# fabriziosestito/policy-server

Measured on AMD Instinct MI355X. Metric: admission requests evaluated/sec (node) at 64 policies; HBM GB/s vs peak, higher is better.
Workload: dtype u8; 1 GPU; C4: 1000000 synthetic Pod AdmissionReviews per GPU x 64 compiled policies (c4_64.yml: 22 psp-capabilities, 21 psp-apparmor, 21 safe-labels); config=c4_64, total_requests=1000000, policies=64, parallelism=dp1 (request shards)

## Files before the change

include/kwgpu.h:

```cpp
#ifndef KWGPU_H
#define KWGPU_H

#include <stddef.h>
#include <stdint.h>

#ifdef __cplusplus
extern "C" {
#endif

enum {
  KW_OK = 0,
  KW_E_INVALID_ID = 1,
  KW_E_INIT = 2,
  KW_E_NOT_FOUND = 3,
  KW_E_BOOTSTRAP = 4,
  KW_E_ENGINE = 5,
  KW_E_GROUP_REHYDRATE = 6,
  KW_E_ARG = 16,
  KW_E_PAYLOAD = 17,
  KW_E_DEVICE = 18,
  KW_E_NOSPACE = 19
};

enum { KW_MODE_PROTECT = 0, KW_MODE_MONITOR = 1 };
// ... 106 lines not shown
int kw_env_pattern_count(const kw_env *env, int col);
int kw_env_pattern(const kw_env *env, int col, int idx, int *kind, char *buf, size_t cap);
int kw_env_classify(const kw_env *env, int col, const char *key, size_t klen, const char *s, size_t len,
                    uint32_t *pats, int cap);

typedef struct kw_batch kw_batch;

int kw_batch_from_json(const char *const *docs, const size_t *lens, size_t n, int doc_kind,
                       kw_batch **out, int64_t *bad_row, char *err, size_t errlen);
int kw_batch_from_soa(const kw_soa *soa, kw_batch **out);
int kw_batch_view(const kw_batch *b, kw_soa *view);
int kw_batch_to_device(kw_batch *b, int device);
int kw_batch_to_device_async(kw_batch *b, int device, void *stream);
int kw_stream_create(int device, void **stream);
void kw_stream_destroy(void *stream);
void kw_batch_destroy(kw_batch *b);

int kw_debug_host_walk(const kw_env *env, const kw_batch *b, const int32_t *policies, uint32_t npol,
                       int origin, uint32_t *out);

int kw_debug_plan(const kw_env *env, kw_batch *b, const int32_t *policies, uint32_t npol, int origin, uint32_t *out,
                  int cap);

int kw_debug_reorder(const kw_batch *b, uint64_t *perm, size_t cap, uint64_t *split, kw_batch **out);

int kw_validate_batch(const kw_env *env, kw_batch *b, const int32_t *policies, uint32_t npol,
                      int origin, void *stream);
int kw_validate_rows(const kw_env *env, kw_batch *b, const int32_t *row_policy, int origin,
                     void *stream);
int kw_batch_verdicts(kw_batch *b, uint32_t *host_out, size_t count);
int kw_validate_host(const kw_env *env, kw_batch *b, const int32_t *policies, uint32_t npol, int origin,
                     int device, uint32_t *out, size_t count, uint32_t chunk_rows);
int kw_batch_pin_host(kw_batch *b, int device);
int kw_host_alloc(int device, size_t bytes, void **out);
void kw_host_free(void *p);
int kw_batch_wide_arg(const kw_batch *b, uint64_t row, int32_t policy, uint64_t *value);
int kw_batch_group_causes(const kw_batch *b, uint64_t row, int32_t policy, uint32_t verdict, uint64_t *words,
                          size_t nwords, size_t *needed);

typedef struct kw_timing {
  double classify_ms;
  double evaluate_ms;
  double total_ms;
  double classify_bytes;
  double evaluate_bytes;
} kw_timing;
// ... 33 lines not shown
```

policy-server_amd/csrc/capi.cpp:

```cpp
#include <hip/hip_runtime.h>

#include <algorithm>
#include <cstdio>
#include <cstdlib>
#include <cstring>
#include <memory>
#include <string>
#include <thread>
#include <vector>

#include "../../include/kwgpu.h"
#include "automaton.hpp"
#include "batch.hpp"
#include "devbatch.hpp"
#include "env.hpp"
#include "kernels.hpp"
#include "knobs.hpp"
#include "metrics.hpp"
#include "pass.hpp"
#include "plan.hpp"
#include "service.hpp"
#include "slotplan.hpp"
#include "upload.hpp"
#include "yaml.hpp"
// ... 512 lines not shown
  std::unique_ptr<DeviceBatch> saved = std::move(kb->dev);
  kb->dev = host_view(kb);
  PassPlan plan;
  int rc = plan_pass(env, kb, policies, npol, nullptr, origin, Knobs::on<KW_BULK_DEBUG>(), &plan);
  const TileArgs& T = plan.geom;
  const uint32_t vals[8] = {T.lds_bytes, (uint32_t)plan.launches.size(), (uint32_t)plan.chunks.size(), T.lds_tables,
                            T.rows, T.cmax, T.kmax, T.lmax};
  for (int i = 0; i < 8; ++i) out[i] = rc == KW_OK ? vals[i] : 0u;
  if (cap >= 16) {
    const bool two = rc == KW_OK && plan.regions.size() == 2;
    const TileArgs* H = two ? &plan.regions[1].geom : nullptr;
    uint32_t more[8] = {rc == KW_OK ? (uint32_t)plan.regions.size() : 0u, (uint32_t)kb->dev->split,
                              rc == KW_OK ? plan.regions[0].grid : 0u, H ? H->lds_bytes : 0u, H ? H->rows : 0u,
                              H ? H->cmax : 0u, two ? plan.regions[1].grid : 0u, 0u};
    if (rc == KW_OK)
      for (size_t k = 0; k < plan.regions.size() && k < 32; ++k) more[7] |= (plan.regions[k].geom.feat & kFeatRng) ? 1u << k : 0u;
    for (int i = 0; i < 8; ++i) out[8 + i] = more[i];
  }
  kb->dev->verdicts = nullptr;
  kb->dev = std::move(saved);
  return rc;
}

int kw_debug_reorder(const kw_batch* kb, uint64_t* perm, size_t cap, uint64_t* split, kw_batch** out) {
  if (!kb || !split || !out || (!perm && kb->b.n) || cap < kb->b.n) return KW_E_ARG;
  std::vector<uint64_t> p;
  *split = split_rows(kb->b, &p);
  if (!*split) {
    p.resize(kb->b.n);
    for (uint64_t r = 0; r < kb->b.n; ++r) p[r] = r;
  }
  auto nb = std::make_unique<kw_batch>();
  RowOrder o;
  permute_batch(kb->b, p, &nb->b, true, &o);
  std::copy(p.begin(), p.end(), perm);
  *out = nb.release();
  return KW_OK;
}

int kw_batch_group_causes(const kw_batch* b, uint64_t row, int32_t policy, uint32_t verdict, uint64_t* words,
                          size_t nwords, size_t* needed) {
  if (!b || (!words && nwords)) return KW_E_ARG;
  if (KW_REASON(verdict) != KW_R_GROUP) return KW_E_ARG;
  const WideData& W = b->b.wide;
  uint32_t bw = 0;
  const uint64_t* big = W.lookup_big(row, policy, &bw);
// ... 128 lines not shown
```

policy-server_amd/csrc/kernels.hip:

```cpp
#include <hip/hip_runtime.h>

#include <algorithm>
#include <array>
#include <cstddef>
#include <mutex>

#include "../../include/kwgpu.h"
#include "imgscan.hpp"
#include "kernels.hpp"


namespace kw {

typedef uint32_t u32x4 __attribute__((ext_vector_type(4)));

__device__ inline uint32_t lit_word(const uint32_t* base, uint32_t i, uint32_t sh, uint32_t len) {
  const uint32_t w = align_bytes(base[i + 1], base[i], sh);
  const uint32_t rem = len - 4u * i;
  return rem >= 4u ? w : (w & ((1u << (8u * rem)) - 1u));
}

template <bool BATCH, int N = 8>
__device__ inline uint32_t lit_lookup(const uint8_t* rec, const uint8_t* bytes, uint32_t b, uint32_t e) {
  const DevLit* L = (const DevLit*)rec;
// ... 337 lines not shown
  x |= (first + 8u <= i) ? y : 0ull;
  y = dpp64<0x142, 0xa>(x);
  x |= (first + r + 1u <= i) ? y : 0ull;
  y = dpp64<0x143, 0xc>(x);
  x |= (lane >= 32u && first + lane - 31u <= i) ? y : 0ull;
  y = dpp64<0x138, 0xf>(x);
  return (first + 1u <= i) ? y : 0ull;
}

template <class T>
__device__ inline const __attribute__((address_space(1))) T* gp(const T* p) {
  return (const __attribute__((address_space(1))) T*)p;
}

__device__ inline uint32_t rup64(uint32_t n) { return (n + 63u) & ~63u; }

__device__ inline uint32_t str_g0(int m, uint32_t r0, uint32_t cb, uint32_t kab, uint32_t kdb, uint32_t lb) {
  return m == S_NS ? r0 : m == S_CAPADD ? kab : m == S_CAPDROP ? kdb : (m == S_LK || m == S_LV) ? lb : cb;
}
__device__ inline uint32_t str_n(int m, uint32_t nr, uint32_t nc, uint32_t nka, uint32_t nkd, uint32_t nl) {
  return m == S_NS ? nr : m == S_CAPADD ? nka : m == S_CAPDROP ? nkd : (m == S_LK || m == S_LV) ? nl : nc;
}

__device__ inline void glds_dwords(const uint32_t* src, uint32_t* dst, uint32_t n, uint32_t tid) {
  const uint32_t lane = tid & 63u;
  for (uint32_t i = tid; i < n; i += kSlotThreads)
    __builtin_amdgcn_global_load_lds((const __attribute__((address_space(1))) void*)(src + i),
                                     (__attribute__((address_space(3))) void*)(dst + (i - lane)), 4, 0, 0);
}
__device__ inline void glds_x4(const u32x4* src, u32x4* dst, uint32_t n, uint32_t tid) {
  const uint32_t lane = tid & 63u;
  for (uint32_t i = tid; i < n; i += kSlotThreads)
    __builtin_amdgcn_global_load_lds((const __attribute__((address_space(1))) void*)(src + i),
                                     (__attribute__((address_space(3))) void*)(dst + (i - lane)), 16, 0, 0);
}
__device__ inline void wglds_dwords(const uint32_t* src, uint32_t* dst, uint32_t n, uint32_t lane) {
  for (uint32_t i = lane; i < n; i += 64u)
    __builtin_amdgcn_global_load_lds((const __attribute__((address_space(1))) void*)(src + i),
                                     (__attribute__((address_space(3))) void*)(dst + (i - lane)), 4, 0, 0);
}
__device__ inline void wglds_x4(const u32x4* src, u32x4* dst, uint32_t n, uint32_t lane) {
  for (uint32_t i = lane; i < n; i += 64u)
    __builtin_amdgcn_global_load_lds((const __attribute__((address_space(1))) void*)(src + i),
                                     (__attribute__((address_space(3))) void*)(dst + (i - lane)), 16, 0, 0);
}

__device__ inline void lds_barrier() { asm volatile("s_waitcnt lgkmcnt(0)\n\ts_barrier" ::: "memory"); }

__device__ inline void prefetch_l2(const void* src, uint32_t bytes, uint8_t* scratch, uint32_t tid) {
  const uint8_t* p = (const uint8_t*)src;
  if ((tid & 63u) >= kPfLanes) return;
  const uint32_t q = (tid >> 6) * kPfLanes + (tid & (kPfLanes - 1u));
// ... 108 lines not shown
  uint32_t* l_cadd = (uint32_t*)region(t.o_cadd);
  uint32_t* l_cdrop = (uint32_t*)region(t.o_cdrop);
  uint16_t* c_ns = (uint16_t*)region(t.o_ns);
  uint16_t* c_aa = (uint16_t*)region(t.o_aa);
  uint16_t* c_img = (uint16_t*)region(t.o_img);
  uint16_t* c_add = (uint16_t*)region(t.o_capadd);
  uint16_t* c_drop = (uint16_t*)region(t.o_capdrop);
  uint16_t* c_lk = (uint16_t*)region(t.o_lk);
  uint16_t* c_lv = (uint16_t*)region(t.o_lv);
  uint64_t* l_rej = (uint64_t*)region(t.o_rej);
  uint64_t* l_mut = (uint64_t*)region(t.o_mut);
  uint8_t* l_byp = region(t.o_byp);
  uint32_t* l_sa = (uint32_t*)region(t.o_sa);
  uint64_t* l_vadd = (uint64_t*)region(t.o_vadd);
  uint64_t* l_vl = (uint64_t*)region(t.o_vl);
  uint64_t* l_vc = (uint64_t*)region(t.o_vc);
  uint64_t* l_vtr = (uint64_t*)region(t.o_vtr);
  uint32_t* l_vw = (uint32_t*)region(t.o_vw);
  uint8_t* own_c = region(t.o_own_c);
  uint8_t* own_l = region(t.o_own_l);
  const ImgLayout il = t.il;
  const uint32_t nim = il.n(), nlv = t.nlv;
  const uint32_t need = t.need;

  if (!desc_early) {
    if (tile < t_hi) fetch_desc(tile, 0);
    __syncthreads();
  }
  mark(4);
  for (uint32_t it = 0; tile < t_hi; ++it) {
    const uint64_t p0_t0 = timing ? clock64() : 0;
    const uint32_t cur = it & 1u;
    uint32_t nxt2 = 0;
    if (dyn && tid == 0) nxt2 = atomicAdd(cnt, 1u);
    if (next < t_hi) fetch_desc(next, cur ^ 1u);
    const TileDesc& d = l_desc[cur];
#define KW_DF(x) sfield(x)
    if (!KW_DF(d.fits)) {
      if (dyn && tid == 0) l_nx[cur] = nxt2;
      __syncthreads();
      tile = next;
      next = dyn ? dbase + l_nx[cur] : next + wpx;
      continue;
    }
    const uint64_t r0 = ((uint64_t)KW_DF(d.r0hi) << 32) | KW_DF(d.r0lo);
    const uint32_t nr = KW_DF(d.nr);
    const uint32_t cb = KW_DF(d.cb), ce = KW_DF(d.ce), lb = KW_DF(d.lb), le = KW_DF(d.le);
    const uint32_t kab = KW_DF(d.kab), kae = KW_DF(d.kae), kdb = KW_DF(d.kdb), kde = KW_DF(d.kde);
    const uint32_t nc = ce - cb, nl = le - lb;
    uint64_t p0_t1 = 0, p0_t2 = 0;
    if (timing) {
      p0_t1 = clock64();
      sg_add(SG_P0_TOP, p0_t1 - p0_t0);
    }

    constexpr bool p0_spread = (LBL || CTR);
    if constexpr (p0_spread) {
      auto job = [&](uint32_t j) { return wave == (j & 3u); };
      if (job(0)) wglds_dwords((const uint32_t*)(a.req_flags + r0), (uint32_t*)l_rf, (nr + 3u) >> 2, lane);
      if (job(1)) wglds_dwords(a.ctr_off + r0, l_coff, nr + 1, lane);
      if (job(2)) wglds_dwords(a.lbl_off + r0, l_loff, nr + 1, lane);
      if (job(3)) wglds_dwords((const uint32_t*)a.ctr_flags + (cb >> 2), (uint32_t*)l_cflags, ((ce + 3u) >> 2) - (cb >> 2), lane);
      if (job(4)) wglds_dwords(a.capadd_off + cb, l_cadd, nc + 1, lane);
      if (job(5)) wglds_dwords(a.capdrop_off + cb, l_cdrop, nc + 1, lane);
      if (timing) {
        p0_t2 = clock64();
        sg_add(SG_P0_REQ, p0_t2 - p0_t1);
      }
#pragma unroll
      for (int m = 0; m < (int)NSTR; ++m) {
        const uint32_t jo = 6u + 2u * (uint32_t)m, jb = jo + 1u;
        if (!(job(jo) || job(jb)) || !t.o_sb[m]) continue;
        if (job(jo)) {
          const uint32_t g0 = str_g0(m, (uint32_t)r0, cb, kab, kdb, lb);
          const uint32_t n = str_n(m, nr, nc, kae - kab, kde - kdb, nl);
          wglds_dwords(t.s_off[m] + g0, (uint32_t*)(lds + t.o_so[m]), n + 1, lane);
        } else {
          wglds_x4((const u32x4*)(t.s_bytes[m] + KW_DF(d.sa[m])), (u32x4*)(lds + t.o_sb[m]), KW_DF(d.nv[m]), lane);
        }
      }
    } else {
      glds_dwords((const uint32_t*)(a.req_flags + r0), (uint32_t*)l_rf, (nr + 3u) >> 2, tid);
      glds_dwords(a.ctr_off + r0, l_coff, nr + 1, tid);
      glds_dwords(a.lbl_off + r0, l_loff, nr + 1, tid);
      glds_dwords((const uint32_t*)a.ctr_flags + (cb >> 2), (uint32_t*)l_cflags, ((ce + 3u) >> 2) - (cb >> 2), tid);
      glds_dwords(a.capadd_off + cb, l_cadd, nc + 1, tid);
      glds_dwords(a.capdrop_off + cb, l_cdrop, nc + 1, tid);
      if (timing) {
        p0_t2 = clock64();
        sg_add(SG_P0_REQ, p0_t2 - p0_t1);
      }
#pragma unroll
      for (int m = 0; m < (int)NSTR; ++m) {
        if (!t.o_sb[m]) continue;
        const uint32_t g0 = str_g0(m, (uint32_t)r0, cb, kab, kdb, lb);
        const uint32_t n = str_n(m, nr, nc, kae - kab, kde - kdb, nl);
        glds_dwords(t.s_off[m] + g0, (uint32_t*)(lds + t.o_so[m]), n + 1, tid);
        glds_x4((const u32x4*)(t.s_bytes[m] + KW_DF(d.sa[m])), (u32x4*)(lds + t.o_sb[m]), KW_DF(d.nv[m]), tid);
      }
    }
    if (timing) sg_add(SG_P0_STR, clock64() - p0_t2);
    for (uint32_t i = tid; i < nr; i += kSlotThreads) l_rej[i] = l_mut[i] = 0;
    if (DYNB && tid == 0) l_nx[2] = l_nx[3] = 0;
    if (tid < NSTR) l_sa[tid] = d.sa[tid];
#undef KW_DF
    const uint64_t p0_end = timing ? clock64() : 0;
    __syncthreads();
    if (timing) sg_add(SG_P0_WAIT, clock64() - p0_end);
    mark(0);
    if (timing && tid == 0) ++ph[5];
    if (dyn && tid == 0) l_nx[cur] = nxt2;
    auto prefetch_next = [&]() {
      if (KW_PREFETCH && LDST && IMG && t.prefetch && next < t_hi) {
        const TileDesc& dn = l_desc[cur ^ 1u];
        if (sfield(dn.fits)) {
          const uint64_t q0 = ((uint64_t)sfield(dn.r0hi) << 32) | sfield(dn.r0lo);
          const uint32_t qn = sfield(dn.nr), qcb = sfield(dn.cb), qc = sfield(dn.ce) - qcb;
          const uint32_t qlb = sfield(dn.lb), qkab = sfield(dn.kab), qkdb = sfield(dn.kdb);
          uint8_t* scratch = lds + t.o_pf;
          prefetch_l2(a.req_flags + q0, qn, scratch, tid);
          prefetch_l2(a.ctr_off + q0, (qn + 1) * 4u, scratch, tid);
          prefetch_l2(a.lbl_off + q0, (qn + 1) * 4u, scratch, tid);
          prefetch_l2(a.ctr_flags + qcb, qc, scratch, tid);
          prefetch_l2(a.capadd_off + qcb, (qc + 1) * 4u, scratch, tid);
// ... 962 lines not shown
```

policy-server_amd/csrc/kernels.hpp:

```cpp
#pragma once
#include <hip/hip_runtime.h>

#include <cstdint>

#include "kwdev.hpp"
#include "slots.hpp"

namespace kw {

enum Str : uint32_t { S_NS = 0, S_IMG, S_AA, S_CAPADD, S_CAPDROP, S_LK, S_LV, NSTR };

struct WideRec {
  uint32_t row_lo, row_hi, policy, value;
};

struct EvalArgs {
  const uint8_t* blob;
  uint64_t nrows;
  uint64_t ndesc;
  uint32_t npol;
  int32_t origin;
  const uint8_t* req_flags;
  const uint32_t* ctr_off;
  const uint32_t* lbl_off;
// ... 30 lines not shown
constexpr uint32_t lds_workgroups_per_cu(uint32_t bytes) {
  const uint32_t g = (bytes + kLdsGranule - 1) / kLdsGranule;
  return g ? kLdsGranules / g : kLdsGranules;
}
constexpr uint32_t kFeatImg = 1, kFeatLbl = 2, kFeatCtr = 4, kFeatGrp = 8, kFeatAll = 15;
constexpr uint32_t kFeatNfa = 16;
constexpr uint32_t kFeatRng = 32;
#ifndef KW_PREFETCH
#define KW_PREFETCH 1
#endif
#ifndef KW_PF_LANES
#define KW_PF_LANES 64
#endif
constexpr uint32_t kPfLanes = KW_PF_LANES;
constexpr uint32_t kMaxChunks = 8;

struct ChunkArgs {
  const uint8_t* rec;
  uint32_t o_lds;
  uint32_t col0, ncols, vec4;
  uint64_t init;
};

struct TileArgs {
  uint32_t rows;
  uint32_t cmax, kmax, lmax;
  uint32_t o_rf, o_coff, o_loff, o_cflags, o_cadd, o_cdrop;
  uint32_t o_ns, o_aa, o_img, o_capadd, o_capdrop, o_lk, o_lv;
  ImgLayout il;
  uint32_t nlv;
  uint32_t need;
  uint32_t o_vadd, o_vl, o_vc, o_vtr;
  uint32_t o_own_c, o_own_l;
  uint32_t o_rej, o_mut, o_byp;
  uint32_t o_nx;
  uint32_t o_desc;
  uint32_t o_pf;
  uint32_t prefetch;
  uint32_t feat;
  uint32_t ctr_ranges;
  uint32_t o_sa;
  uint32_t o_vw, vw_stride;
  uint32_t o_so[NSTR], o_sb[NSTR], sb_cap[NSTR];
  const uint32_t* s_off[NSTR];
  const uint8_t* s_bytes[NSTR];
  uint32_t lds_tables;
  uint32_t lit_lds[NCOL], dfa_lds[NCOL], kv_lds;
  uint32_t lit_blob[NCOL], dfa_blob[NCOL], kv_blob, nlk;
  uint32_t nstage;
  uint32_t stage_blob[NCOL + kMaxChunks], stage_lds[NCOL + kMaxChunks], stage_bytes[NCOL + kMaxChunks];
  uint32_t bypass_cls, docker_io_cls, latest_cls;
  uint32_t nchunk;
  ChunkArgs chunk[kMaxChunks];
  uint32_t rows_mode;
  uint32_t debug;
  uint32_t lds_bytes;
};

struct alignas(16) TileDesc {
  uint32_t cb, ce, lb, le, kab, kae, kdb, kde;
  uint32_t sa[NSTR];
  uint32_t pad0;
  uint32_t nv[NSTR];
  uint32_t fits;
  uint32_t r0lo, r0hi, nr;
  uint32_t pad[4];
};
static_assert(sizeof(TileDesc) == 128, "TileDesc layout");

hipError_t launch_evaluate_tiles(const EvalArgs& a, const TileArgs& t, const TileArgs* d_t, const TileDesc* d_desc,
                                 uint32_t grid, hipStream_t s);
struct WideGroupArgs {
  uint32_t prog_off, prog_len;
  uint32_t col;
  uint32_t nmem, midx_off;
  uint32_t okw, rejb;
  uint32_t cause_off, cause_words;
  uint32_t errw;
  uint32_t kind;
  uint32_t mutw;
};

constexpr uint32_t kSplitMember = 0x80000000u;

template <class Part>
KW_HD inline uint32_t combine_parts(const WideGroupArgs& g, const uint32_t* part_off, Part part) {
  bool mutated = false;
  for (uint32_t s = 0; s < g.nmem; ++s) {
    const uint32_t x = part(s);
    if (!(x & KW_V_ALLOWED)) {
      uint32_t reason = KW_REASON(x), arg = KW_ARG(x);
// ... 55 lines not shown
```

policy-server_amd/csrc/pass.cpp:

```cpp
#include "pass.hpp"

#include <atomic>
#include <chrono>
#include <cstdio>
#include <cstring>
#include <memory>

#include "knobs.hpp"
#include "plan.hpp"

namespace kw {

int upload_env(kw_env* env, int device) {
  if (device < 0) return KW_OK;
  HIPCHK(hipSetDevice(device));
  HIPCHK(hipMalloc(&env->e.d_blob, env->e.blob.size()));
  HIPCHK(hipMemcpy(env->e.d_blob, env->e.blob.data(), env->e.blob.size(), hipMemcpyHostToDevice));
  env->e.device = device;
  return KW_OK;
}

int build_descs(const Batch& B, const TileArgs& T, uint64_t lo, uint64_t hi, uint64_t t0, uint64_t t1, uint64_t range,
                std::vector<TileDesc>* desc, std::vector<uint32_t>* ovf) {
  auto make = [&](uint64_t r0, uint64_t r1, TileDesc* dp) {
// ... 246 lines not shown
  D.last_nwide = plan.nwide;
  D.last_wide_policy = plan.wide_policy;
  D.last_rows_mode = plan.rows_mode;
  D.last_row_words = plan.args.npol;
  D.last_wide_cap = A.wide_cap;
  *out_args = A;
  return KW_OK;
}

static void print_phase_report(size_t launch, uint32_t grid, const std::vector<uint64_t>& ph) {
  double sum[kPhaseWords] = {0};
  for (uint32_t g = 0; g < grid; ++g)
    for (uint32_t k = 0; k < kPhaseWords; ++k) sum[k] += (double)ph[(size_t)g * kPhaseWords + k];
  const double tiles = std::max(1.0, sum[5]);
  fprintf(stderr,
          "[kw phase] launch %zu grid %u tiles %.0f: cycles/tile P0 %.0f P1 %.0f D %.0f P2 %.0f P3+next %.0f "
          "(sum %.0f); per workgroup: %.0f cycles, %.2f tiles, table staging %.0f\n",
          launch, grid, tiles, sum[0] / tiles, sum[1] / tiles, sum[2] / tiles, sum[3] / tiles, sum[4] / tiles,
          (sum[0] + sum[1] + sum[2] + sum[3] + sum[4]) / tiles, sum[6] / grid, tiles / grid, sum[7] / grid);
  const double wt = tiles * (double)(kSlotThreads / 64u);
  const double* g = sum + 8;
  fprintf(stderr,
          "[kw seg] per wave-tile: P0 wait %.0f | P1 busy %.0f wait %.0f (label %.0f capstr %.0f ctr %.0f image %.0f req %.0f) "
          "| P2 busy %.0f wait %.0f (ctr %.0f label %.0f req %.0f) | P3 busy %.0f wait %.0f | P0 issue: top %.0f "
          "request arrays %.0f strings %.0f\n",
          g[SG_P0_WAIT] / wt, g[SG_P1_BUSY] / wt, g[SG_P1_WAIT] / wt, g[SG_P1_LABEL] / wt, g[SG_P1_CAPSTR] / wt,
          g[SG_P1_CTR] / wt, g[SG_P1_IMAGE] / wt, g[SG_P1_REQ] / wt, g[SG_P2_BUSY] / wt, g[SG_P2_WAIT] / wt,
          g[SG_P2_CTR] / wt, g[SG_P2_LABEL] / wt, g[SG_P2_REQ] / wt, g[SG_P3_BUSY] / wt, g[SG_P3_WAIT] / wt,
          g[SG_P0_TOP] / wt, g[SG_P0_REQ] / wt, g[SG_P0_STR] / wt);
  const uint32_t nx = std::min(8u, grid);
  uint32_t late = 0;
  double spread = 0;
  for (uint32_t x = 0; x < nx; ++x) {
    std::vector<uint64_t> st;
    for (uint32_t q = x; q < grid; q += nx) st.push_back(ph[(size_t)q * kPhaseWords + 8 + SG_START]);
    std::sort(st.begin(), st.end());
    for (uint64_t v : st) late += v > st[0] + 2000;
    spread = std::max(spread, (double)(st.back() - st[0]) / 100.0);
  }
  fprintf(stderr, "[kw start] launch %zu: %u of %u workgroups started > 20 us after their XCD's first (widest spread %.1f us)\n",
          launch, late, grid, spread);
}

static int run_pass(kw_batch* kb, PassPlan& plan, bool timed, hipStream_t s) {
  DeviceBatch& D = *kb->dev;
  EvalArgs A;
  if (int rc = prepare_pass(kb, plan, s, &A)) return rc;
  const bool phases = (plan.geom.debug & 512u) != 0;
// ... 272 lines not shown
```

policy-server_amd/csrc/plan.cpp:

```cpp
#define KW_PLANNING_TU
#include "plan.hpp"

#include <algorithm>
#include <chrono>
#include <cstdio>
#include <cstring>
#include <map>

#include "knobs.hpp"
#include "slots.hpp"

namespace kw {

bool sched_dynamic(uint64_t ntiles, uint32_t grid, bool lds_tables) {
  const char* e = PlanKnobs::str<KW_SCHED>();
  if (!strcmp(e, "static")) return false;
  if (!strcmp(e, "dynamic")) return true;
  return ntiles > (lds_tables ? 16ull : 4ull) * std::max<uint32_t>(grid, 1);
}

namespace {

uint32_t heavy_rows() { return (uint32_t)PlanKnobs::num<KW_HEAVY_ROWS>(); }

// ... 543 lines not shown
      T.stage_blob[T.nstage] = stages[k].blob;
      T.stage_lds[T.nstage] = lds_at[k];
      T.stage_bytes[T.nstage] = (stages[k].bytes + 15u) & ~15u;
      ++T.nstage;
    }
  for (int c = 0; c < (int)NCOL; ++c) {
    if (P.lit_of[c]) {
      T.lit_blob[c] = stages[P.lit_of[c] - 1].blob;
      T.lit_lds[c] = lds_at[P.lit_of[c] - 1];
    }
    if (P.dfa_of[c]) {
      T.dfa_blob[c] = stages[P.dfa_of[c] - 1].blob;
      T.dfa_lds[c] = lds_at[P.dfa_of[c] - 1];
    }
  }
  if (P.kv_stage) {
    T.kv_blob = stages[P.kv_stage - 1].blob;
    T.kv_lds = ldst ? lds_at[P.kv_stage - 1] : 0u;
  } else if (need & (1u << S_LV)) {
    T.kv_blob = H->kv_off;
    T.kv_lds = 0;
  }
  T.debug = debug;
}

void dump_plan(const TileArgs& T, const PassNeeds& N, const TablePlan& P, size_t nchunks, size_t nlaunches) {
  fprintf(stderr, "[kw tile] lds_tables=%u rows=%u cmax=%u kmax=%u lmax=%u lds=%u area=%u (classifiers %u) chunks=%zu launches=%zu nim=%u nlv=%u\n",
          T.lds_tables, T.rows, T.cmax, T.kmax, T.lmax, T.lds_bytes, P.area, P.table_bytes, nchunks, nlaunches, N.il.n(), N.nlv);
  for (size_t k = 0; k < P.stages.size(); ++k) fprintf(stderr, "[kw tile]   classifier stage %zu: %u bytes\n", k, P.stages[k].bytes);
  uint32_t so = 0, sb = 0;
  for (int m = 0; m < (int)NSTR; ++m)
    if (T.o_sb[m]) so += T.o_sb[m] - T.o_so[m], sb += T.sb_cap[m] + 48;
  fprintf(stderr,
          "[kw tile]   layout: headers %u | classes ns %u aa %u img %u caps %u lk %u lv %u | sets vadd %u vl %u vc %u vtr %u | "
          "owners %u | rej/mut/byp %u | union at %u: string offsets %u + bytes %u, violation words %u | total %u\n",
          T.o_ns - T.o_rf, T.o_aa - T.o_ns, T.o_img - T.o_aa, T.o_capadd - T.o_img, T.o_lk - T.o_capadd, T.o_lv - T.o_lk,
          T.o_vadd - T.o_lv, T.o_vl - T.o_vadd, T.o_vc - T.o_vl, T.o_vtr - T.o_vc, T.o_own_c - T.o_vtr, T.o_rej - T.o_own_c,
          T.o_sa - T.o_rej, T.o_vw, so, sb, T.rows * T.vw_stride * 4, T.lds_bytes);
}

void plan_launch_args(const TablePlan& P, uint32_t npol, PassPlan* plan) {
  plan->slot_blob.clear();
  plan->slot_at.clear();
  for (const SlotChunk& c : plan->chunks) {
    plan->slot_at.push_back((uint32_t)plan->slot_blob.size());
    plan->slot_blob.insert(plan->slot_blob.end(), c.rec.begin(), c.rec.end());
// ... 32 lines not shown
  A.lbl_off = D.lbl_off;
  A.ctr_flags = D.ctr_flags;
  A.capadd_off = D.capadd_off;
  A.capdrop_off = D.capdrop_off;
  A.out = D.verdicts;
  A.nwide = plan->nwide;
  plan->wide_cap_per_row = plan->rows_mode ? 1u : npol;
  if (!A.req_flags || !A.ctr_off || !A.lbl_off || !A.ctr_flags || !A.capadd_off || !A.capdrop_off || !A.out) return KW_E_ARG;
  for (int m = 0; m < (int)NSTR; ++m)
    if ((N.need & (1u << m)) && (!plan->geom.s_off[m] || !plan->geom.s_bytes[m])) return KW_E_ARG;

  const double n = (double)B.n;
  double eb = n * (1 + 4 + 4) + 4.0 * n * (double)A.npol;
  if (N.any_ctr) eb += (double)B.containers() * 1.0;
  if (N.any_caps) eb += (double)B.containers() * 8.0;
  for (int m = 0; m < (int)NSTR; ++m)
    if (N.need & (1u << m)) eb += (double)D.str[m].nbytes + 4.0 * (double)D.str[m].n;
  plan->evaluate_bytes = eb;
  return KW_OK;
}

}

int plan_pass(const kw_env* env, kw_batch* kb, const int32_t* pols, uint32_t npol, const int32_t* row_policy,
              int origin, bool timing, PassPlan* plan) {
  const Env& E = env->e;
  DeviceBatch& D = *kb->dev;
  const Batch& B = dev_rows(kb);
  const DevHeader* H = (const DevHeader*)E.blob.data();
  plan->env_blob = E.blob.data();
  plan->rows_mode = row_policy != nullptr;
  const uint32_t debug = (uint32_t)PlanKnobs::num<KW_TILE_DEBUG>();
  const auto pt0 = std::chrono::steady_clock::now();
  auto pms = [&]() { return std::chrono::duration<double, std::milli>(std::chrono::steady_clock::now() - pt0).count(); };

  if (int rc = plan_columns(E, B, D, pols, npol, row_policy, origin, plan)) return rc;
  const double t_slots = timing ? pms() : 0.0;
  const PassNeeds N = classify_chunks(plan->chunks, H);
  const TablePlan P = plan_tables(H, N.need, plan->chunks, &plan->launches);

  const TileCtx C{B, D, N, P.area, (debug & 256u) != 0};
  std::vector<std::pair<uint64_t, uint64_t>> bounds{{0, B.n}};
  if (D.split && D.split < B.n) bounds = {{0, D.split}, {D.split, B.n}};
  plan->regions.clear();
  for (const auto& [lo, hi] : bounds) {
    const DeviceBatch::RowsPlan& pick = pick_rows(C, lo, hi);
// ... 18 lines not shown
```

policy-server_amd/kwgpu/__init__.py:

```python
import ctypes as C
import json

from . import _native as N
from ._native import KwSoa, KwTiming

PROTECT, MONITOR = N.KW_MODE_PROTECT, N.KW_MODE_MONITOR
VALIDATE, AUDIT = N.KW_ORIGIN_VALIDATE, N.KW_ORIGIN_AUDIT


class RequestOrigin:
    Validate = N.KW_ORIGIN_VALIDATE
    Audit = N.KW_ORIGIN_AUDIT


class PolicyMode:
    Protect = N.KW_MODE_PROTECT
    Monitor = N.KW_MODE_MONITOR


class EvaluationError(Exception):

    code = None

    def __init__(self, message, code=None):
# ... 325 lines not shown
    def validate_host(self, env, policies, out=None, origin=VALIDATE, device=0, chunk_rows=0):
        import numpy as np
        npol = len(policies)
        count = self.n * npol
        if out is None:
            out = np.empty(count, dtype=np.uint32)
        elif out.dtype != np.uint32 or not out.flags.c_contiguous or out.size < count:
            raise ValueError("out must be a contiguous uint32 array of at least rows x policies words")
        arr = (C.c_int32 * npol)(*[env._idx(p) for p in policies])
        rc = self._L.kw_validate_host(env._h, self._h, arr, npol, origin, device,
                                      out.ctypes.data_as(C.POINTER(C.c_uint32)), count, chunk_rows)
        raise_for(rc, "kw_validate_host failed")
        self.device = device
        self._npol = npol
        return out[:count]

    def debug_plan(self, env, policies, origin=VALIDATE):
        arr = env._array(policies)
        out = (C.c_uint32 * 16)()
        raise_for(self._L.kw_debug_plan(env._h, self._h, arr, len(policies), origin, out, 16), "kw_debug_plan failed")
        keys = ("lds_bytes", "launches", "chunks", "lds_tables", "rows", "cmax", "kmax", "lmax", "regions", "split",
                "grid", "heavy_lds_bytes", "heavy_rows", "heavy_cmax", "heavy_grid", "scan_regions")
        return dict(zip(keys, out[:16]))

    def debug_reorder(self):
        import numpy as np
        perm = np.zeros(max(self.n, 1), dtype=np.uint64)
        split, h = C.c_uint64(), C.c_void_p()
        rc = self._L.kw_debug_reorder(self._h, perm.ctypes.data_as(C.POINTER(C.c_uint64)), len(perm), C.byref(split),
                                      C.byref(h))
        raise_for(rc, "kw_debug_reorder failed")
        return Batch(h.value), perm[:self.n], split.value

    def wide_arg(self, row, policy):
        v = C.c_uint64()
        rc = self._L.kw_batch_wide_arg(self._h, row, policy, C.byref(v))
        return v.value if rc == N.KW_OK else None

    def group_causes(self, row, policy, verdict):
        need = C.c_size_t()
        words = (C.c_uint64 * 1)()
        rc = self._L.kw_batch_group_causes(self._h, row, policy, int(verdict), words, 1, C.byref(need))
        if rc == N.KW_E_NOSPACE:
            words = (C.c_uint64 * need.value)()
            rc = self._L.kw_batch_group_causes(self._h, row, policy, int(verdict), words, need.value, C.byref(need))
        raise_for(rc, "kw_batch_group_causes")
# ... 197 lines not shown
```

policy-server_amd/kwgpu/_native.py:

```python
import ctypes as C
import os

PKG_DIR = os.path.dirname(os.path.dirname(os.path.abspath(__file__)))
LIB_PATH = os.environ.get("KWGPU_LIB") or os.path.join(PKG_DIR, "libkwgpu.so")
SYNTH_PATH = os.path.join(PKG_DIR, "libkwsynth.so")

KW_OK = 0
KW_E_INVALID_ID = 1
KW_E_INIT = 2
KW_E_NOT_FOUND = 3
KW_E_BOOTSTRAP = 4
KW_E_ENGINE = 5
KW_E_GROUP_REHYDRATE = 6
KW_E_ARG = 16
KW_E_PAYLOAD = 17
KW_E_DEVICE = 18
KW_E_NOSPACE = 19

KW_MODE_PROTECT = 0
KW_MODE_MONITOR = 1
KW_ORIGIN_VALIDATE = 0
KW_ORIGIN_AUDIT = 1
KW_DOC_ADMISSION_REVIEW = 0
KW_DOC_RAW_REVIEW = 1
# ... 31 lines not shown
        ("capadd_off", C.POINTER(C.c_uint32)),
        ("capdrop_off", C.POINTER(C.c_uint32)),
        ("ctr_name", KwStrcol), ("ctr_image", KwStrcol), ("ctr_apparmor", KwStrcol),
        ("cap_add", KwStrcol), ("cap_drop", KwStrcol),
        ("lbl_key", KwStrcol), ("lbl_val", KwStrcol),
    ]


class KwEnvOptions(C.Structure):
    _fields_ = [("continue_on_errors", C.c_int), ("always_accept_namespace", C.c_char_p), ("device", C.c_int)]


class KwTiming(C.Structure):
    _fields_ = [("classify_ms", C.c_double), ("evaluate_ms", C.c_double), ("total_ms", C.c_double),
                ("classify_bytes", C.c_double), ("evaluate_bytes", C.c_double)]


EXPORTS = [
    "kw_env_build", "kw_env_build_yaml", "kw_yaml_to_json", "kw_env_serialize", "kw_env_deserialize", "kw_env_destroy", "kw_env_lookup",
    "kw_env_policy_count", "kw_env_policy_id", "kw_env_is_group", "kw_env_get_policy_mode",
    "kw_env_get_policy_allowed_to_mutate",
    "kw_env_should_always_accept_requests_made_inside_of_namespace",
    "kw_env_policy_initialization_error", "kw_env_validate_settings", "kw_pattern_match", "kw_pattern_match_many", "kw_env_pattern_count",
    "kw_env_pattern", "kw_env_classify", "kw_batch_wide_arg", "kw_batch_group_causes", "kw_debug_plan", "kw_debug_reorder",
    "kw_batch_from_json", "kw_batch_from_soa", "kw_batch_view", "kw_batch_to_device", "kw_batch_to_device_async",
    "kw_stream_create", "kw_stream_destroy", "kw_validate_host", "kw_batch_pin_host", "kw_host_alloc", "kw_host_free",
    "kw_batch_destroy", "kw_debug_host_walk", "kw_validate_batch", "kw_validate_rows", "kw_batch_verdicts",
    "kw_validate_timed", "kw_format_response", "kw_format_response_doc", "kw_env_group_members", "kw_evaluate",
    "kw_service_constraints", "kw_metrics_create", "kw_metrics_destroy", "kw_metrics_record", "kw_metrics_render",
    "kw_metrics_reset", "kw_version",
]

_lib = None
_synth = None


def lib():
    global _lib
    if _lib is not None:
        return _lib
    if not os.path.exists(LIB_PATH):
        raise ImportError(f"{LIB_PATH} is missing: run __graft_entry__.build() (hipcc --offload-arch=gfx950)")
    try:
        import torch
    except ImportError:
        pass
    L = C.CDLL(LIB_PATH)
# ... 3 lines not shown
        "kw_env_build": (ip, [cp, sz, C.POINTER(KwEnvOptions), C.POINTER(vp), cp, sz]),
        "kw_env_build_yaml": (ip, [cp, sz, C.POINTER(KwEnvOptions), C.POINTER(vp), cp, sz]),
        "kw_yaml_to_json": (ip, [cp, sz, cp, sz, C.POINTER(sz)]),
        "kw_env_serialize": (ip, [vp, vp, sz, C.POINTER(sz)]),
        "kw_env_deserialize": (ip, [vp, sz, ip, C.POINTER(vp), cp, sz]),
        "kw_env_destroy": (None, [vp]),
        "kw_env_lookup": (ip, [vp, cp, sz, C.POINTER(i32)]),
        "kw_env_policy_count": (ip, [vp]),
        "kw_env_policy_id": (ip, [vp, i32, cp, sz]),
        "kw_env_is_group": (ip, [vp, i32]),
        "kw_env_get_policy_mode": (ip, [vp, i32, C.POINTER(ip)]),
        "kw_env_get_policy_allowed_to_mutate": (ip, [vp, i32, C.POINTER(ip)]),
        "kw_env_should_always_accept_requests_made_inside_of_namespace": (ip, [vp, cp, sz]),
        "kw_env_policy_initialization_error": (ip, [vp, i32, cp, sz]),
        "kw_env_validate_settings": (ip, [vp, i32, cp, sz]),
        "kw_pattern_match": (ip, [ip, cp, cp, sz]),
        "kw_pattern_match_many": (ip, [ip, cp, C.POINTER(cp), C.POINTER(sz), sz, C.POINTER(C.c_int32)]),
        "kw_env_pattern_count": (ip, [vp, ip]),
        "kw_env_pattern": (ip, [vp, ip, ip, C.POINTER(ip), cp, sz]),
        "kw_env_classify": (ip, [vp, ip, cp, sz, cp, sz, C.POINTER(u32), ip]),
        "kw_batch_wide_arg": (ip, [vp, u64, i32, C.POINTER(u64)]),
        "kw_batch_group_causes": (ip, [vp, u64, i32, C.c_uint32, C.POINTER(u64), C.c_size_t, C.POINTER(C.c_size_t)]),
        "kw_debug_plan": (ip, [vp, vp, C.POINTER(i32), u32, ip, C.POINTER(u32), ip]),
        "kw_debug_reorder": (ip, [vp, C.POINTER(u64), sz, C.POINTER(u64), C.POINTER(vp)]),
        "kw_batch_from_json": (ip, [C.POINTER(cp), C.POINTER(sz), sz, ip, C.POINTER(vp), C.POINTER(C.c_int64), cp, sz]),
        "kw_batch_from_soa": (ip, [C.POINTER(KwSoa), C.POINTER(vp)]),
        "kw_batch_view": (ip, [vp, C.POINTER(KwSoa)]),
        "kw_batch_to_device": (ip, [vp, ip]),
        "kw_batch_to_device_async": (ip, [vp, ip, vp]),
        "kw_stream_create": (ip, [ip, C.POINTER(vp)]),
        "kw_stream_destroy": (None, [vp]),
        "kw_batch_destroy": (None, [vp]),
        "kw_validate_batch": (ip, [vp, vp, C.POINTER(i32), u32, ip, vp]),
        "kw_validate_rows": (ip, [vp, vp, C.POINTER(i32), ip, vp]),
        "kw_batch_verdicts": (ip, [vp, C.POINTER(u32), sz]),
        "kw_validate_host": (ip, [vp, vp, C.POINTER(i32), u32, ip, ip, C.POINTER(u32), sz, u32]),
        "kw_batch_pin_host": (ip, [vp, ip]),
        "kw_host_alloc": (ip, [ip, sz, C.POINTER(vp)]),
        "kw_host_free": (None, [vp]),
        "kw_debug_host_walk": (ip, [vp, vp, C.POINTER(i32), u32, ip, C.POINTER(u32)]),
        "kw_validate_timed": (ip, [vp, vp, C.POINTER(i32), u32, ip, ip, ip, C.POINTER(KwTiming)]),
        "kw_format_response": (ip, [vp, vp, u64, i32, u32, C.POINTER(u32), cp, sz, C.POINTER(sz)]),
        "kw_format_response_doc": (ip, [vp, vp, u64, i32, u32, C.POINTER(u32), cp, sz, ip, cp, sz, C.POINTER(sz)]),
        "kw_env_group_members": (ip, [vp, i32, C.POINTER(i32), ip]),
        "kw_evaluate": (ip, [vp, cp, cp, sz, ip, ip, cp, sz, C.POINTER(sz)]),
        "kw_service_constraints": (ip, [u32, ip, ip, C.POINTER(u32)]),
# ... 37 lines not shown
```

Measured before the change: 4.010 billion requests/s.

## Drive tile LDS staging from a host-built copy-job table spread across waves

Replaces the hard-coded per-column global-to-LDS copy sequence in the tile kernel with a table of copy jobs built on the host. Each job holds a base pointer and a packed code from which the kernel derives span offset and count. Jobs are sorted by trip count and assigned round-robin to waves, with readlane broadcasting per-job parameters. This aims to balance phase-0 copy issue across waves for every kernel variant, not only the label/container ones. It adds per-tile span arithmetic and a larger TileArgs, plus a debug API to dump the job plan.

```diff
diff --git a/include/kwgpu.h b/include/kwgpu.h
--- a/include/kwgpu.h
+++ b/include/kwgpu.h
@@ -152,6 +152,9 @@
 int kw_debug_plan(const kw_env *env, kw_batch *b, const int32_t *policies, uint32_t npol, int origin, uint32_t *out,
                   int cap);
 
+int kw_debug_copy_jobs(const kw_env *env, kw_batch *b, const int32_t *policies, uint32_t npol, int origin,
+                       uint32_t *out, size_t cap, size_t *needed);
+
 int kw_debug_reorder(const kw_batch *b, uint64_t *perm, size_t cap, uint64_t *split, kw_batch **out);
 
 int kw_validate_batch(const kw_env *env, kw_batch *b, const int32_t *policies, uint32_t npol,
diff --git a/policy-server_amd/csrc/capi.cpp b/policy-server_amd/csrc/capi.cpp
--- a/policy-server_amd/csrc/capi.cpp
+++ b/policy-server_amd/csrc/capi.cpp
@@ -558,6 +558,60 @@
   return rc;
 }
 
+int kw_debug_copy_jobs(const kw_env* env, kw_batch* kb, const int32_t* policies, uint32_t npol, int origin, uint32_t* out,
+                       size_t cap, size_t* needed) {
+  if (!env || !kb || !needed || (!out && cap) || (!policies && npol)) return KW_E_ARG;
+  std::unique_ptr<DeviceBatch> saved = std::move(kb->dev);
+  kb->dev = host_view(kb);
+  const DeviceBatch& D = *kb->dev;
+  const Batch& B = dev_rows(kb);
+  PassPlan plan;
+  int rc = plan_pass(env, kb, policies, npol, nullptr, origin, false, &plan);
+  std::vector<uint32_t> w;
+  if (rc == KW_OK) {
+    const void* cols[kMaxCopyJobs] = {D.req_flags, D.ctr_off, D.lbl_off, D.ctr_flags, D.capadd_off, D.capdrop_off};
+    for (int m = 0; m < (int)NSTR; ++m) cols[6 + 2 * m] = D.str[m].off, cols[7 + 2 * m] = D.str[m].bytes;
+    w.push_back((uint32_t)plan.regions.size());
+    for (const PassPlan::Region& rg : plan.regions) {
+      const TileArgs& T = rg.geom;
+      std::vector<TileDesc> desc;
+      std::vector<uint32_t> ovf;
+      const uint64_t ntiles = (rg.hi - rg.lo + T.rows - 1) / T.rows;
+      if ((rc = build_descs(B, T, rg.lo, rg.hi, 0, ntiles, 4096, &desc, &ovf))) break;
+      for (uint32_t v : {T.rows, T.njobs, (uint32_t)desc.size(), (uint32_t)ovf.size(), (uint32_t)rg.lo, (uint32_t)rg.hi, T.lds_bytes,
+                         (uint32_t)D.split})
+        w.push_back(v);
+      for (uint32_t v : {T.o_rf, T.o_coff, T.o_loff, T.o_cflags, T.o_cadd, T.o_cdrop}) w.push_back(v);
+      w.insert(w.end(), T.o_so, T.o_so + NSTR);
+      w.insert(w.end(), T.o_sb, T.o_sb + NSTR);
+      for (uint32_t j = 0; j < T.njobs; ++j) {
+        const CopyJob& q = T.jobs[j];
+        uint32_t col = 0xffffffffu;
+        for (uint32_t c = 0; c < kMaxCopyJobs; ++c)
+          if ((c < 6 || T.o_sb[(c - 6) / 2]) && q.base == (uint64_t)(uintptr_t)cols[c] && col == 0xffffffffu) col = c;
+        for (uint32_t v : {col, copy_lds(q.code), (q.code & kCjX4) ? 16u : 4u, q.code}) w.push_back(v);
+      }
+      for (const TileDesc& d : desc) {
+        const uint32_t* dw = (const uint32_t*)&d;
+        w.insert(w.end(), dw, dw + sizeof(TileDesc) / 4);
+        for (uint32_t j = 0; j < T.njobs; ++j) {
+          const uint32_t code = T.jobs[j].code;
+          const CopySpan sp = copy_span(code, dw[code & 31u], dw[(code >> 5) & 31u], d.r0hi);
+          for (uint32_t v : {(uint32_t)sp.byte_off, (uint32_t)(sp.byte_off >> 32), sp.count}) w.push_back(v);
+        }
+      }
+      w.insert(w.end(), ovf.begin(), ovf.end());
+    }
+  }
+  kb->dev->verdicts = nullptr;
+  kb->dev = std::move(saved);
+  if (rc) return rc;
+  *needed = w.size();
+  if (cap < w.size()) return KW_E_NOSPACE;
+  std::copy(w.begin(), w.end(), out);
+  return KW_OK;
+}
+
 int kw_debug_reorder(const kw_batch* kb, uint64_t* perm, size_t cap, uint64_t* split, kw_batch** out) {
   if (!kb || !split || !out || (!perm && kb->b.n) || cap < kb->b.n) return KW_E_ARG;
   std::vector<uint64_t> p;
diff --git a/policy-server_amd/csrc/kernels.hip b/policy-server_amd/csrc/kernels.hip
--- a/policy-server_amd/csrc/kernels.hip
+++ b/policy-server_amd/csrc/kernels.hip
@@ -383,12 +383,6 @@
   return m == S_NS ? nr : m == S_CAPADD ? nka : m == S_CAPDROP ? nkd : (m == S_LK || m == S_LV) ? nl : nc;
 }
 
-__device__ inline void glds_dwords(const uint32_t* src, uint32_t* dst, uint32_t n, uint32_t tid) {
-  const uint32_t lane = tid & 63u;
-  for (uint32_t i = tid; i < n; i += kSlotThreads)
-    __builtin_amdgcn_global_load_lds((const __attribute__((address_space(1))) void*)(src + i),
-                                     (__attribute__((address_space(3))) void*)(dst + (i - lane)), 4, 0, 0);
-}
 __device__ inline void glds_x4(const u32x4* src, u32x4* dst, uint32_t n, uint32_t tid) {
   const uint32_t lane = tid & 63u;
   for (uint32_t i = tid; i < n; i += kSlotThreads)
@@ -543,6 +537,14 @@
   const ImgLayout il = t.il;
   const uint32_t nim = il.n(), nlv = t.nlv;
   const uint32_t need = t.need;
+  const uint32_t njobs = t.njobs;
+  uint32_t jb_lo = 0, jb_hi = 0, jb_code = 0;
+  if (lane < njobs) {
+    const CopyJob q = tp->jobs[lane];
+    jb_lo = (uint32_t)q.base;
+    jb_hi = (uint32_t)(q.base >> 32);
+    jb_code = q.code;
+  }
 
   if (!desc_early) {
     if (tile < t_hi) fetch_desc(tile, 0);
@@ -564,63 +566,41 @@
       next = dyn ? dbase + l_nx[cur] : next + wpx;
       continue;
     }
+    uint64_t p0_t1 = 0, p0_t2 = 0;
+    if (timing) {
+      p0_t1 = clock64();
+      sg_add(SG_P0_TOP, p0_t1 - p0_t0);
+    }
+
+    {
+      const uint32_t* dw = (const uint32_t*)&d;
+      uint32_t code_v = jb_code;
+      asm volatile("" : "+v"(code_v));
+      const CopySpan sp = copy_span(code_v, dw[code_v & 31u], dw[(code_v >> 5) & 31u], d.r0hi);
+      const uint64_t src = (((uint64_t)jb_hi << 32) | jb_lo) + sp.byte_off;
+      const uint32_t s_lo = (uint32_t)src, s_hi = (uint32_t)(src >> 32);
+      if (timing) {
+        p0_t2 = clock64();
+        sg_add(SG_P0_REQ, p0_t2 - p0_t1);
+      }
+      for (uint32_t j = wave; j < njobs; j += kSlotThreads / 64u) {
+        const uint64_t p = ((uint64_t)(uint32_t)__builtin_amdgcn_readlane((int)s_hi, (int)j) << 32) |
+                           (uint32_t)__builtin_amdgcn_readlane((int)s_lo, (int)j);
+        const uint32_t n = (uint32_t)__builtin_amdgcn_readlane((int)sp.count, (int)j);
+        const uint32_t code = (uint32_t)__builtin_amdgcn_readlane((int)code_v, (int)j);
+        uint8_t* dst = lds + copy_lds(code);
+        if (code & kCjX4)
+          wglds_x4((const u32x4*)p, (u32x4*)dst, n, lane);
+        else
+          wglds_dwords((const uint32_t*)p, (uint32_t*)dst, n, lane);
+      }
+    }
     const uint64_t r0 = ((uint64_t)KW_DF(d.r0hi) << 32) | KW_DF(d.r0lo);
     const uint32_t nr = KW_DF(d.nr);
     const uint32_t cb = KW_DF(d.cb), ce = KW_DF(d.ce), lb = KW_DF(d.lb), le = KW_DF(d.le);
     const uint32_t kab = KW_DF(d.kab), kae = KW_DF(d.kae), kdb = KW_DF(d.kdb), kde = KW_DF(d.kde);
+    if (timing) sg_add(SG_P0_STR, clock64() - p0_t2);
     const uint32_t nc = ce - cb, nl = le - lb;
-    uint64_t p0_t1 = 0, p0_t2 = 0;
-    if (timing) {
-      p0_t1 = clock64();
-      sg_add(SG_P0_TOP, p0_t1 - p0_t0);
-    }
-
-    constexpr bool p0_spread = (LBL || CTR);
-    if constexpr (p0_spread) {
-      auto job = [&](uint32_t j) { return wave == (j & 3u); };
-      if (job(0)) wglds_dwords((const uint32_t*)(a.req_flags + r0), (uint32_t*)l_rf, (nr + 3u) >> 2, lane);
-      if (job(1)) wglds_dwords(a.ctr_off + r0, l_coff, nr + 1, lane);
-      if (job(2)) wglds_dwords(a.lbl_off + r0, l_loff, nr + 1, lane);
-      if (job(3)) wglds_dwords((const uint32_t*)a.ctr_flags + (cb >> 2), (uint32_t*)l_cflags, ((ce + 3u) >> 2) - (cb >> 2), lane);
-      if (job(4)) wglds_dwords(a.capadd_off + cb, l_cadd, nc + 1, lane);
-      if (job(5)) wglds_dwords(a.capdrop_off + cb, l_cdrop, nc + 1, lane);
-      if (timing) {
-        p0_t2 = clock64();
-        sg_add(SG_P0_REQ, p0_t2 - p0_t1);
-      }
-#pragma unroll
-      for (int m = 0; m < (int)NSTR; ++m) {
-        const uint32_t jo = 6u + 2u * (uint32_t)m, jb = jo + 1u;
-        if (!(job(jo) || job(jb)) || !t.o_sb[m]) continue;
-        if (job(jo)) {
-          const uint32_t g0 = str_g0(m, (uint32_t)r0, cb, kab, kdb, lb);
-          const uint32_t n = str_n(m, nr, nc, kae - kab, kde - kdb, nl);
-          wglds_dwords(t.s_off[m] + g0, (uint32_t*)(lds + t.o_so[m]), n + 1, lane);
-        } else {
-          wglds_x4((const u32x4*)(t.s_bytes[m] + KW_DF(d.sa[m])), (u32x4*)(lds + t.o_sb[m]), KW_DF(d.nv[m]), lane);
-        }
-      }
-    } else {
-      glds_dwords((const uint32_t*)(a.req_flags + r0), (uint32_t*)l_rf, (nr + 3u) >> 2, tid);
-      glds_dwords(a.ctr_off + r0, l_coff, nr + 1, tid);
-      glds_dwords(a.lbl_off + r0, l_loff, nr + 1, tid);
-      glds_dwords((const uint32_t*)a.ctr_flags + (cb >> 2), (uint32_t*)l_cflags, ((ce + 3u) >> 2) - (cb >> 2), tid);
-      glds_dwords(a.capadd_off + cb, l_cadd, nc + 1, tid);
-      glds_dwords(a.capdrop_off + cb, l_cdrop, nc + 1, tid);
-      if (timing) {
-        p0_t2 = clock64();
-        sg_add(SG_P0_REQ, p0_t2 - p0_t1);
-      }
-#pragma unroll
-      for (int m = 0; m < (int)NSTR; ++m) {
-        if (!t.o_sb[m]) continue;
-        const uint32_t g0 = str_g0(m, (uint32_t)r0, cb, kab, kdb, lb);
-        const uint32_t n = str_n(m, nr, nc, kae - kab, kde - kdb, nl);
-        glds_dwords(t.s_off[m] + g0, (uint32_t*)(lds + t.o_so[m]), n + 1, tid);
-        glds_x4((const u32x4*)(t.s_bytes[m] + KW_DF(d.sa[m])), (u32x4*)(lds + t.o_sb[m]), KW_DF(d.nv[m]), tid);
-      }
-    }
-    if (timing) sg_add(SG_P0_STR, clock64() - p0_t2);
     for (uint32_t i = tid; i < nr; i += kSlotThreads) l_rej[i] = l_mut[i] = 0;
     if (DYNB && tid == 0) l_nx[2] = l_nx[3] = 0;
     if (tid < NSTR) l_sa[tid] = d.sa[tid];
diff --git a/policy-server_amd/csrc/kernels.hpp b/policy-server_amd/csrc/kernels.hpp
--- a/policy-server_amd/csrc/kernels.hpp
+++ b/policy-server_amd/csrc/kernels.hpp
@@ -76,6 +76,33 @@
   uint64_t init;
 };
 
+struct CopyJob {
+  uint64_t base;
+  uint32_t code;
+  uint32_t pad;
+};
+constexpr uint32_t kCjRel = 1u << 10, kCjReq = 1u << 11, kCjQuad = 1u << 12, kCjAlign = 1u << 13, kCjPlus1 = 1u << 14,
+                   kCjElem4 = 1u << 15, kCjX4 = 1u << 16, kCjLdsShift = 18;
+constexpr uint32_t copy_code(uint32_t wb, uint32_t we, uint32_t lds, uint32_t flags) {
+  return wb | (we << 5) | flags | ((lds >> 4) << kCjLdsShift);
+}
+KW_HD constexpr uint32_t copy_lds(uint32_t code) { return (code >> kCjLdsShift) << 4; }
+struct CopySpan {
+  uint64_t byte_off;
+  uint32_t count;
+};
+KW_HD inline CopySpan copy_span(uint32_t code, uint32_t b, uint32_t e, uint32_t r0hi) {
+  const uint32_t sh = (code >> 11) & 2u, bsh = (code >> 14) & 2u, rnd = (1u << sh) - 1u;
+  const uint32_t rel = 0u - ((code >> 10) & 1u), req = 0u - ((code >> 11) & 1u), al = 0u - ((code >> 13) & 1u);
+  const uint32_t b0 = b & ~(rnd & al);
+  const uint32_t end = e + (b & rel);
+  CopySpan s;
+  s.count = ((end - b0 + rnd) >> sh) + ((code >> 14) & 1u);
+  s.byte_off = (((uint64_t)(r0hi & req) << 32) | b0) << bsh;
+  return s;
+}
+constexpr uint32_t kMaxCopyJobs = 6 + 2 * NSTR;
+
 struct TileArgs {
   uint32_t rows;
   uint32_t cmax, kmax, lmax;
@@ -98,6 +125,8 @@
   uint32_t o_so[NSTR], o_sb[NSTR], sb_cap[NSTR];
   const uint32_t* s_off[NSTR];
   const uint8_t* s_bytes[NSTR];
+  CopyJob jobs[kMaxCopyJobs];
+  uint32_t njobs;
   uint32_t lds_tables;
   uint32_t lit_lds[NCOL], dfa_lds[NCOL], kv_lds;
   uint32_t lit_blob[NCOL], dfa_blob[NCOL], kv_blob, nlk;
@@ -121,6 +150,8 @@
   uint32_t pad[4];
 };
 static_assert(sizeof(TileDesc) == 128, "TileDesc layout");
+
+void build_copy_jobs(TileArgs* T, const void* const cols[6]);
 
 hipError_t launch_evaluate_tiles(const EvalArgs& a, const TileArgs& t, const TileArgs* d_t, const TileDesc* d_desc,
                                  uint32_t grid, hipStream_t s);
diff --git a/policy-server_amd/csrc/pass.cpp b/policy-server_amd/csrc/pass.cpp
--- a/policy-server_amd/csrc/pass.cpp
+++ b/policy-server_amd/csrc/pass.cpp
@@ -292,8 +292,8 @@
   const double* g = sum + 8;
   fprintf(stderr,
           "[kw seg] per wave-tile: P0 wait %.0f | P1 busy %.0f wait %.0f (label %.0f capstr %.0f ctr %.0f image %.0f req %.0f) "
-          "| P2 busy %.0f wait %.0f (ctr %.0f label %.0f req %.0f) | P3 busy %.0f wait %.0f | P0 issue: top %.0f "
-          "request arrays %.0f strings %.0f\n",
+          "| P2 busy %.0f wait %.0f (ctr %.0f label %.0f req %.0f) | P3 busy %.0f wait %.0f | P0 issue: top to fits %.0f "
+          "job spans %.0f job loop %.0f\n",
           g[SG_P0_WAIT] / wt, g[SG_P1_BUSY] / wt, g[SG_P1_WAIT] / wt, g[SG_P1_LABEL] / wt, g[SG_P1_CAPSTR] / wt,
           g[SG_P1_CTR] / wt, g[SG_P1_IMAGE] / wt, g[SG_P1_REQ] / wt, g[SG_P2_BUSY] / wt, g[SG_P2_WAIT] / wt,
           g[SG_P2_CTR] / wt, g[SG_P2_LABEL] / wt, g[SG_P2_REQ] / wt, g[SG_P3_BUSY] / wt, g[SG_P3_WAIT] / wt,
diff --git a/policy-server_amd/csrc/plan.cpp b/policy-server_amd/csrc/plan.cpp
--- a/policy-server_amd/csrc/plan.cpp
+++ b/policy-server_amd/csrc/plan.cpp
@@ -589,6 +589,8 @@
     T.kv_lds = 0;
   }
   T.debug = debug;
+  const void* const cols[6] = {D.req_flags, D.ctr_off, D.lbl_off, D.ctr_flags, D.capadd_off, D.capdrop_off};
+  build_copy_jobs(&T, cols);
 }
 
 void dump_plan(const TileArgs& T, const PassNeeds& N, const TablePlan& P, size_t nchunks, size_t nlaunches) {
@@ -667,6 +669,48 @@
 
 }
 
+void build_copy_jobs(TileArgs* Tp, const void* const cols[6]) {
+  TileArgs& T = *Tp;
+  constexpr uint32_t W_CB = offsetof(TileDesc, cb) / 4, W_CE = offsetof(TileDesc, ce) / 4, W_LB = offsetof(TileDesc, lb) / 4,
+                     W_LE = offsetof(TileDesc, le) / 4, W_KAB = offsetof(TileDesc, kab) / 4, W_KAE = offsetof(TileDesc, kae) / 4,
+                     W_KDB = offsetof(TileDesc, kdb) / 4, W_KDE = offsetof(TileDesc, kde) / 4, W_SA = offsetof(TileDesc, sa) / 4,
+                     W_NV = offsetof(TileDesc, nv) / 4, W_R0 = offsetof(TileDesc, r0lo) / 4, W_NR = offsetof(TileDesc, nr) / 4;
+  static_assert(W_NR < 32 && offsetof(TileDesc, r0hi) / 4 == W_R0 + 1, "copy_code holds 5-bit descriptor words");
+  struct Todo {
+    CopyJob j;
+    uint32_t trips;
+  };
+  std::vector<Todo> todo;
+  auto add = [&](const void* base, uint32_t code, uint32_t pieces) {
+    todo.push_back({{(uint64_t)(uintptr_t)base, code, 0u}, (pieces + 63u) / 64u});
+  };
+  const uint32_t req = kCjRel | kCjReq, offs = kCjElem4 | kCjPlus1;
+  add(cols[0], copy_code(W_R0, W_NR, T.o_rf, req | kCjQuad), (T.rows + 3) / 4);
+  add(cols[1], copy_code(W_R0, W_NR, T.o_coff, req | offs), T.rows + 1);
+  add(cols[2], copy_code(W_R0, W_NR, T.o_loff, req | offs), T.rows + 1);
+  add(cols[3], copy_code(W_CB, W_CE, T.o_cflags, kCjQuad | kCjAlign), (T.cmax + 3) / 4 + 1);
+  add(cols[4], copy_code(W_CB, W_CE, T.o_cadd, offs), T.cmax + 1);
+  add(cols[5], copy_code(W_CB, W_CE, T.o_cdrop, offs), T.cmax + 1);
+  for (uint32_t m = 0; m < NSTR; ++m) {
+    if (!T.o_sb[m]) continue;
+    uint32_t wb = W_CB, we = W_CE, fl = offs, cap = T.cmax;
+    if (m == S_NS) wb = W_R0, we = W_NR, fl |= req, cap = T.rows;
+    else if (m == S_CAPADD) wb = W_KAB, we = W_KAE, cap = T.kmax;
+    else if (m == S_CAPDROP) wb = W_KDB, we = W_KDE, cap = T.kmax;
+    else if (m == S_LK || m == S_LV) wb = W_LB, we = W_LE, cap = T.lmax;
+    add(T.s_off[m], copy_code(wb, we, T.o_so[m], fl), cap + 1);
+    add(T.s_bytes[m], copy_code(W_SA + m, W_NV + m, T.o_sb[m], kCjRel | kCjX4), T.sb_cap[m] / 16);
+  }
+  std::stable_sort(todo.begin(), todo.end(), [](const Todo& a, const Todo& b) { return a.trips > b.trips; });
+  memset(T.jobs, 0, sizeof(T.jobs));
+  T.njobs = (uint32_t)todo.size();
+  for (uint32_t k = 0; k < T.njobs; ++k) {
+    const uint32_t row = k / 4u, i = k % 4u;
+    const uint32_t len = std::min(4u, T.njobs - row * 4u);
+    T.jobs[row * 4u + ((row & 1u) ? len - 1u - i : i)] = todo[k].j;
+  }
+}
+
 int plan_pass(const kw_env* env, kw_batch* kb, const int32_t* pols, uint32_t npol, const int32_t* row_policy,
               int origin, bool timing, PassPlan* plan) {
   const Env& E = env->e;
diff --git a/policy-server_amd/kwgpu/__init__.py b/policy-server_amd/kwgpu/__init__.py
--- a/policy-server_amd/kwgpu/__init__.py
+++ b/policy-server_amd/kwgpu/__init__.py
@@ -371,6 +371,19 @@
         keys = ("lds_bytes", "launches", "chunks", "lds_tables", "rows", "cmax", "kmax", "lmax", "regions", "split",
                 "grid", "heavy_lds_bytes", "heavy_rows", "heavy_cmax", "heavy_grid", "scan_regions")
         return dict(zip(keys, out[:16]))
+
+    def debug_copy_jobs(self, env, policies, origin=VALIDATE):
+        import numpy as np
+        arr = env._array(policies)
+        need = C.c_size_t()
+        rc = self._L.kw_debug_copy_jobs(env._h, self._h, arr, len(policies), origin, None, 0, C.byref(need))
+        if rc != N.KW_E_NOSPACE:
+            raise_for(rc, "kw_debug_copy_jobs failed")
+        out = np.zeros(max(need.value, 1), dtype=np.uint32)
+        rc = self._L.kw_debug_copy_jobs(env._h, self._h, arr, len(policies), origin,
+                                        out.ctypes.data_as(C.POINTER(C.c_uint32)), out.size, C.byref(need))
+        raise_for(rc, "kw_debug_copy_jobs failed")
+        return out[:need.value]
 
     def debug_reorder(self):
         import numpy as np
diff --git a/policy-server_amd/kwgpu/_native.py b/policy-server_amd/kwgpu/_native.py
--- a/policy-server_amd/kwgpu/_native.py
+++ b/policy-server_amd/kwgpu/_native.py
@@ -77,7 +77,7 @@
     "kw_env_get_policy_allowed_to_mutate",
     "kw_env_should_always_accept_requests_made_inside_of_namespace",
     "kw_env_policy_initialization_error", "kw_env_validate_settings", "kw_pattern_match", "kw_pattern_match_many", "kw_env_pattern_count",
-    "kw_env_pattern", "kw_env_classify", "kw_batch_wide_arg", "kw_batch_group_causes", "kw_debug_plan", "kw_debug_reorder",
+    "kw_env_pattern", "kw_env_classify", "kw_batch_wide_arg", "kw_batch_group_causes", "kw_debug_plan", "kw_debug_copy_jobs", "kw_debug_reorder",
     "kw_batch_from_json", "kw_batch_from_soa", "kw_batch_view", "kw_batch_to_device", "kw_batch_to_device_async",
     "kw_stream_create", "kw_stream_destroy", "kw_validate_host", "kw_batch_pin_host", "kw_host_alloc", "kw_host_free",
     "kw_batch_destroy", "kw_debug_host_walk", "kw_validate_batch", "kw_validate_rows", "kw_batch_verdicts",
@@ -127,6 +127,7 @@
         "kw_batch_wide_arg": (ip, [vp, u64, i32, C.POINTER(u64)]),
         "kw_batch_group_causes": (ip, [vp, u64, i32, C.c_uint32, C.POINTER(u64), C.c_size_t, C.POINTER(C.c_size_t)]),
         "kw_debug_plan": (ip, [vp, vp, C.POINTER(i32), u32, ip, C.POINTER(u32), ip]),
+        "kw_debug_copy_jobs": (ip, [vp, vp, C.POINTER(i32), u32, ip, C.POINTER(u32), sz, C.POINTER(sz)]),
         "kw_debug_reorder": (ip, [vp, C.POINTER(u64), sz, C.POINTER(u64), C.POINTER(vp)]),
         "kw_batch_from_json": (ip, [C.POINTER(cp), C.POINTER(sz), sz, ip, C.POINTER(vp), C.POINTER(C.c_int64), cp, sz]),
         "kw_batch_from_soa": (ip, [C.POINTER(KwSoa), C.POINTER(vp)]),
```

Measured after the change: 4.155 billion requests/s (median of 6 runs). 3.6% higher.
